# ReplayCoding/mt-renderer

Measured on AMD Instinct MI355X. Metric: Mtris/sec, 1M-tri 64-bone skinned scene @1920x1080, higher is better.
Workload: dtype f32; 1 GPU; headline: 20 x mesh50k primitives = 1,000,000 strip triangles, 506,520 vertices x 24 B, 64-bone palette, debug-id shader, 1920x1080; triangles_per_frame=1000000, collective=none

## Files before the change

### mt_renderer_amd/csrc/k_tile.hip

```cpp
#include "tile_common.h"

namespace mtr {

#define TRI_PASS 64
#ifndef FRAG_K
#define FRAG_K 8u
#endif

struct TriC {
    int32_t A0, B0, C0, A1;
    int32_t B1, C1, A2, B2;
    int32_t C2;
    uint32_t flags;
    float z0, dz1;
    float dz2, rcpA;
    uint32_t rgba8;
    uint32_t pad;
};
struct TriX {
    UVPlanes p;
    uint32_t tw, th, tlevels;
    const uint8_t* tex;
    uint64_t pad2;
};
static_assert(sizeof(TriC) == 64 && sizeof(TriX) == 64, "LDS triangle records are 64 B");
enum { TF_LARGE = 1, TF_TEX = 2, TF_BLEND = 4, TF_ADD = 8, TF_NODW = 128, TF_NODT = 256, TF_BLENDSOLID = 512 };

template <bool TEX>
__device__ __forceinline__ void setup_entry(const TileParams& P, uint32_t r, int32_t binx0, int32_t biny0, TriC& t, TriX* x,
                                            int4& chi, uint32_t& submask) {
    const RecA a = load_rec(P.fb, r);
    const bool solid = (a.pad1 & 1u) != 0;
    DMat mat = {};
    if (!solid) mat = P.mats[a.mat];
    const uint32_t mshader = solid ? (uint32_t)MTR_SH_DEBUG : mat.shader;
    const int32_t X[3] = {a.X0, a.X1, a.X2}, Y[3] = {a.Y0, a.Y1, a.Y2};
    TriSetup g;
    tri_setup(X, Y, a.z0, a.z1, a.z2, binx0, biny0, g);
    uint32_t flags = g.flags;
    if (TEX && mshader == MTR_SH_TEXTURED) flags |= TF_TEX;
    if (!solid) {
        if (mat.blend == MTR_DB_ALPHA) flags |= TF_BLEND;
        if (mat.blend == MTR_DB_ADD) flags |= TF_ADD;
        if (!(mat.dstate & 1u)) flags |= TF_NODW;
        if (!(mat.dstate & 2u)) flags |= TF_NODT;
        if (mshader != MTR_SH_TEXTURED && mat.blend == MTR_DB_ADD) flags |= TF_BLENDSOLID;
    }
    t.A0 = g.A[0]; t.B0 = g.B[0]; t.C0 = g.Clo[0];
    t.A1 = g.A[1]; t.B1 = g.B[1]; t.C1 = g.Clo[1];
    t.A2 = g.A[2]; t.B2 = g.B[2]; t.C2 = g.Clo[2];
    t.flags = flags;
    t.z0 = g.z0; t.dz1 = g.dz1; t.dz2 = g.dz2; t.rcpA = g.rcpA;
    t.rgba8 = solid ? a.pad0 : mat.rgba8;
    chi = make_int4(g.Chi[0], g.Chi[1], g.Chi[2], 0);
// ... 31 lines not shown
    } else {
        const QuadUV q = quad();
        const TexRef tr = {Xt.tex, Xt.tw, Xt.th, Xt.tlevels};
        float src[4];
        sample_texture(tr, q.u, q.v, filter_select(q.dudx, q.dvdx, q.dudy, q.dvdy, tr.tw, tr.th, tr.levels), src);
        col = blend_store(col, src, bmode);
    }
}

template <bool TEX>
__global__ __launch_bounds__(64) void k_tile(TileParams P) {
    __shared__ __align__(16) TriC s_tc[TRI_PASS];
    __shared__ __align__(16) TriX s_tx[TEX ? TRI_PASS : 1];
    __shared__ __align__(16) int4 s_chi[TRI_PASS];
    __shared__ uint32_t s_mask[TRI_PASS];
    __shared__ uint32_t s_off[64], s_pre[65];
    __shared__ Seg s_seg[64];
    __shared__ uint32_t s_cnt[MTR_BIN * MTR_BIN];
    __shared__ __align__(16) uint8_t s_frag[MTR_BIN * MTR_BIN * FRAG_K];
    __shared__ unsigned long long s_start[32];
    __shared__ uint32_t s_pm[TRI_PASS];
    __shared__ uint8_t s_tmap[TRI_PASS];

    const uint32_t ovf = tile_prologue(P);
    const uint32_t lane = threadIdx.x;
    uint32_t bin;
    if (!block_to_bin(P, bin)) return;
    if (P.mixed && !P.bin_flag[bin]) return;
    uint32_t bin_x, bin_y;
    bin_xy(P, bin, bin_x, bin_y);
    const int32_t binx0 = (int32_t)bin_x * MTR_BIN, biny0 = (int32_t)bin_y * MTR_BIN;

    float dep[4];
    uint32_t col[4];
#pragma unroll
    for (int i = 0; i < 4; i++) { dep[i] = P.clear_depth; col[i] = P.clear_rgba8; }
    for (uint32_t i = lane; i < MTR_BIN * MTR_BIN; i += 64) s_cnt[i] = 0u;

    uint32_t seg_lo, S, ent_lo, n_ent;
    bin_queue(P.fb, bin, ent_lo, n_ent, seg_lo, S);
    if (ovf) { n_ent = 0; S = 0; }
    if (P.fb.direct && lane == 0 && n_ent) {
        atomicAdd(&P.fb.counters[MTR_CTR(CTR_ENT, bin)], n_ent);
        atomicAdd(&P.fb.counters[MTR_CTR(CTR_SEG, bin)], S);
    }
    const Seg* segs = P.fb.segs + seg_lo;

    unsigned long long lo = 0, hi = 1ull << 32, width = 1ull << 32, end = 1ull << 32;
    if (S > 64) {
        uint32_t kmin = 0xFFFFFFFFu, kmax = 0;
        for (uint32_t i = lane; i < S; i += 64) { const uint32_t k = segs[i].key; kmin = min(kmin, k); kmax = max(kmax, k); }
#pragma unroll
        for (int d = 32; d > 0; d >>= 1) { kmin = min(kmin, (uint32_t)__shfl_xor((int)kmin, d)); kmax = max(kmax, (uint32_t)__shfl_xor((int)kmax, d)); }
        width = ((unsigned long long)(kmax - kmin) + 1) * 40 / S + 1;
        lo = kmin; hi = lo + width; end = (unsigned long long)kmax + 1;
    }
    while (S != 0 && lo < end) {
        uint32_t n;
        uint32_t mkey = 0xFFFFFFFFu, moff = 0, mcnt = 0;
        if (S <= 64) {
            n = S;
            if (lane < S) { const Seg sg = segs[lane]; mkey = sg.key; moff = sg.off; mcnt = sg.cnt; }
        } else {
            uint32_t cnt = 0;
            for (uint32_t i = lane; i < S; i += 64) { const uint32_t k = segs[i].key; cnt += (k >= lo && k < hi) ? 1u : 0u; }
#pragma unroll
            for (int d = 32; d > 0; d >>= 1) cnt += (uint32_t)__shfl_xor((int)cnt, d);
// ... 31 lines not shown
                }
            uint32_t inc = mcnt;
#pragma unroll
            for (int d = 1; d < 64; d <<= 1) {
                const uint32_t t = (uint32_t)__shfl_up((int)inc, d);
                if ((int)lane >= d) inc += t;
            }
            s_off[lane] = moff;
            s_pre[lane] = inc - mcnt;
            if (lane == 63) s_pre[64] = inc;
            wave_lds_sync();
            const uint32_t N = s_pre[64];

            for (uint32_t e0 = 0; e0 < N; e0 += TRI_PASS) {
                const uint32_t cntp = min((uint32_t)TRI_PASS, N - e0);
                if (lane < cntp) {
                    const uint32_t e = e0 + lane;
                    uint32_t a = 0, b = 64;
#pragma unroll
                    for (int it = 0; it < 6; it++) {
                        const uint32_t mid = (a + b) >> 1;
                        if (s_pre[mid] <= e) a = mid; else b = mid;
                    }
                    const uint32_t ord = P.fb.entries[ent_lo + s_off[a] + (e - s_pre[a])];
                    const uint32_t r = (ord >> 7) * MTR_CHUNK_SLOTS + (ord & 127u);
                    setup_entry<TEX>(P, r, binx0, biny0, s_tc[lane], TEX ? &s_tx[lane] : nullptr, s_chi[lane], s_mask[lane]);
                }
                wave_lds_sync();
                bool listed = false;
                {
                    const uint32_t box = lane < cntp ? s_tc[lane].pad : 0u;
                    const uint32_t bw = ((box >> 8) & 15u) + 1u, bh = ((box >> 12) & 15u) + 1u;
                    const uint32_t mine = (box >> 16) ? bw * bh : 0u;
                    const bool large = lane < cntp && (s_tc[lane].flags & TF_LARGE);
                    const uint32_t inc = wave_incl_scan_u32(mine);
                    const uint32_t total = (uint32_t)__builtin_amdgcn_readlane((int)inc, 63);
                    if (!__ballot(large) && total != 0 && total <= 2048u) {
                        const uint32_t pre = inc - mine, cidx = lane_rank(__ballot(mine != 0));
                        flat_stage_starts(s_start, 32, lane, mine, pre);
                        if (mine) {
                            s_tmap[cidx] = (uint8_t)lane;
                            s_pm[lane] = pre | (row_magic(bw) << 12);
                        }
                        wave_lds_sync();
                        flat_for_each(s_start, 32, lane, total, [&](uint32_t pidx, uint32_t ci) {
                            const uint32_t t = s_tmap[ci];
                            const int4* tc = reinterpret_cast<const int4*>(&s_tc[t]);
// ... 7 lines not shown
                            int32_t e1, e2;
                            if (tri_inside(E, lx, ly, e1, e2)) {
                                const uint32_t pix = (uint32_t)(ly * MTR_BIN + lx);
                                const uint32_t slot = atomicAdd(&s_cnt[pix], 1u);
                                if (slot < FRAG_K) s_frag[pix * FRAG_K + slot] = (uint8_t)t;
                            }
                        });
                        wave_lds_sync();
                        uint32_t cn[4];
                        bool over = false;
#pragma unroll
                        for (int i = 0; i < 4; i++) {
                            const uint32_t pix = (uint32_t)(((i >> 1) * 8 + (lane >> 3)) * MTR_BIN + (i & 1) * 8 + (lane & 7));
                            cn[i] = s_cnt[pix];
                            s_cnt[pix] = 0u;
                            over = over || cn[i] > FRAG_K;
                        }
                        if (!__ballot(over)) {
                            listed = true;
#pragma unroll
                            for (int i = 0; i < 4; i++) {
                                const int32_t lx = (int32_t)((i & 1) * 8 + (lane & 7)), ly = (int32_t)((i >> 1) * 8 + (lane >> 3));
                                const uint32_t pix = (uint32_t)(ly * MTR_BIN + lx);
                                const bool in_vp = (uint32_t)(binx0 + lx) < P.fb.W && (uint32_t)(biny0 + ly) < P.fb.H;
                                uint32_t fw[FRAG_K / 4];
#pragma unroll
                                for (uint32_t j = 0; j < FRAG_K / 4; j++) fw[j] = reinterpret_cast<const uint32_t*>(&s_frag[pix * FRAG_K])[j];
                                const uint32_t n = in_vp ? cn[i] : 0u;
                                int32_t last = -1;
                                for (;;) {
                                    uint32_t best = 255u;
#pragma unroll
                                    for (uint32_t j = 0; j < FRAG_K; j++) {
                                        const uint32_t f = (fw[j >> 2] >> (8u * (j & 3u))) & 0xffu;
                                        if (j < n && (int32_t)f > last && f < best) best = f;
                                    }
                                    if (!__ballot(best != 255u)) break;
                                    if (best == 255u) continue;
                                    last = (int32_t)best;
                                    const int4* tc = reinterpret_cast<const int4*>(&s_tc[best]);
                                    const int4 q0 = tc[0], q1 = tc[1], q2 = tc[2], q3 = tc[3];
                                    const uint32_t flags = (uint32_t)q2.y;
                                    const float rcpA = __int_as_float(q3.y);
                                    auto bary = [&](int32_t x, int32_t y, float& b1, float& b2) {
                                        b1 = tri_bary(tri_edge(q1.y, q0.w, q1.x, x, y), (flags >> 5) & 1u, rcpA);
                                        b2 = tri_bary(tri_edge(q2.x, q1.z, q1.w, x, y), (flags >> 6) & 1u, rcpA);
                                    };
                                    float b1, b2;
                                    bary(lx, ly, b1, b2);
                                    const TriX& Xt = s_tx[TEX ? best : 0];
                                    resolve_fragment<TEX>(q2, q3, Xt, true, b1, b2, dep[i], col[i], [&] { return quad_uv(Xt.p, lx, ly, bary); });
                                }
                            }
                        }
                    }
                }
                if (listed) { wave_lds_sync(); continue; }
#pragma unroll
                for (int i = 0; i < 4; i++) {
                    const int32_t lx = (int32_t)((i & 1) * 8 + (lane & 7)), ly = (int32_t)((i >> 1) * 8 + (lane >> 3));
                    const bool in_vp = (uint32_t)(binx0 + lx) < P.fb.W && (uint32_t)(biny0 + ly) < P.fb.H;
                    uint64_t m = __ballot(lane < cntp && ((s_mask[lane] >> i) & 1u));
                    while (m) {
                        const uint32_t t = __builtin_amdgcn_readfirstlane((uint32_t)__ffsll((long long)m) - 1);
                        m &= m - 1;
                        const int4* tc = reinterpret_cast<const int4*>(&s_tc[t]);
                        const int4 q0 = tc[0], q1 = tc[1], q2 = tc[2], q3 = tc[3];
                        const TriEdges E = {q0.x, q0.y, q0.z, q0.w, q1.x, q1.y, q1.z, q1.w, q2.x};
                        const uint32_t flags = (uint32_t)q2.y;
                        const float rcpA = __int_as_float(q3.y);
                        bool inside;
                        float b1, b2;
                        if (!(flags & TF_LARGE)) {
                            int32_t e1, e2;
                            inside = tri_inside(E, lx, ly, e1, e2);
                            b1 = tri_bary(e1, (flags >> 5) & 1u, rcpA);
                            b2 = tri_bary(e2, (flags >> 6) & 1u, rcpA);
                        } else {
                            const int4 ch = s_chi[t];
                            inside = tri_inside_large(E, ch.x, ch.y, ch.z, flags, rcpA, lx, ly, b1, b2);
                        }
                        const TriX& Xt = s_tx[TEX ? t : 0];
                        QuadUV q = {};
                        if (TEX && (flags & TF_TEX)) {
                            uv_at_bary(Xt.p, b1, b2, q.u, q.v);
                            auto across = [&](float a, uint32_t bit) { return __shfl(a, (int)(lane | bit)) - __shfl(a, (int)(lane & ~bit)); };
                            q.dudx = across(q.u, 1u); q.dvdx = across(q.v, 1u);
                            q.dudy = across(q.u, 8u); q.dvdy = across(q.v, 8u);
                        }
                        resolve_fragment<TEX>(q2, q3, Xt, inside && in_vp, b1, b2, dep[i], col[i], [&] { return q; });
                    }
                }
                wave_lds_sync();
            }
        }
        lo = hi;
        hi = lo + width;
        if (hi > (1ull << 32)) hi = 1ull << 32;
    }

    if (lane == 0) bin_queue_done(P.fb, bin);
#pragma unroll
    for (int i = 0; i < 4; i++) {
        const uint32_t x = (uint32_t)binx0 + (i & 1) * 8 + (lane & 7), y = (uint32_t)biny0 + (i >> 1) * 8 + (lane >> 3);
        if (x < P.fb.W && y < P.fb.H) {
            const size_t pi = (size_t)y * P.fb.W + x;
            reinterpret_cast<uint32_t*>(P.color)[pi] = col[i];
            P.depth[pi] = dep[i];
        }
    }
}

}

void mtr_launch_tile(const TileParams& p_in, bool textured, hipStream_t s) {
    TileParams p = p_in;
    tile_set_divisors(p);
    const uint32_t mine = p.fb.own.own_count;
    if (mine == 0) return;
    uint32_t grid = (mine + 7) / 8 * 8;
    if (p.xcd_run) grid = (grid / 8 + p.xcd_run - 1) / p.xcd_run * p.xcd_run * 8;
    if (textured) hipLaunchKernelGGL(mtr::k_tile<true>, dim3(grid), dim3(64), 0, s, p);
    else hipLaunchKernelGGL(mtr::k_tile<false>, dim3(grid), dim3(64), 0, s, p);
}
```

### mt_renderer_amd/csrc/k_tile_vis.hip

```cpp
#include "tile_common.h"

namespace mtr {

struct VisTri {
    int32_t A0, B0, C0, A1;
    int32_t B1, C1, A2, B2;
    int32_t C2;
    uint32_t flags;
    float z0, dz1;
    float dz2, rcpA;
    uint32_t ordk;
    uint32_t box;
};
static_assert(sizeof(VisTri) == 64, "VisTri is 64 B");

struct Setup {
    VisTri t;
    int4 chi;
    int32_t npx;
    uint32_t bhm1;
};

__device__ __forceinline__ void setup_tri(const RecA& a, uint32_t ord, int32_t binx0, int32_t biny0, int32_t vw, int32_t vh, Setup& s) {
    const int32_t X[3] = {a.X0, a.X1, a.X2}, Y[3] = {a.Y0, a.Y1, a.Y2};
// ... 49 lines not shown
__device__ __forceinline__ float z_at(const RecA& a, int32_t px, int32_t py) {
    float b1, b2;
    tri_abs_bary(a.X0, a.Y0, a.X1, a.Y1, a.X2, a.Y2, px, py, b1, b2);
    return tri_depth(b1, b2, a.z0, a.z1 - a.z0, a.z2 - a.z0);
}

#ifndef VIS_OCC
#define VIS_OCC 6
#endif

template <bool TEX, int VIS_WAVES, bool STAIR, bool QW>
__global__ __launch_bounds__(64 * VIS_WAVES, VIS_OCC) void k_tile_vis(TileParams P) {
    __shared__ unsigned long long s_key[MTR_BIN * MTR_BIN];
    __shared__ uint4 s_flat[VIS_WAVES][64 * 4];
    __shared__ unsigned long long s_start[VIS_WAVES][64];
    __shared__ uint32_t s_trans;
    __shared__ uint32_t s_hard;
    __shared__ uint32_t s_cnt[STAIR ? MTR_BIN * MTR_BIN : 1];
    __shared__ __align__(16) uint32_t s_list[STAIR ? MTR_BIN * MTR_BIN * STAIR_K : 4];

    static_assert(!QW, "the quad walk is retired");
    const uint32_t lane = threadIdx.x & 63;
    const uint32_t wv = __builtin_amdgcn_readfirstlane(threadIdx.x >> 6);
    const uint32_t ovf = tile_prologue(P);
    uint32_t bin;
    if (!block_to_bin(P, bin)) return;
    uint32_t bin_x, bin_y;
    bin_xy(P, bin, bin_x, bin_y);
    const int32_t binx0 = (int32_t)bin_x * MTR_BIN, biny0 = (int32_t)bin_y * MTR_BIN;
    const float cd = P.clear_depth;
    const bool zlim_ok = cd >= 0.0f;
    const uint32_t zlim = __float_as_uint(fminf(cd, 1.0f));
    const int32_t vw = (int32_t)P.fb.W - binx0, vh = (int32_t)P.fb.H - biny0;
    const uint32_t stride = 64 * VIS_WAVES, first = wv * 64;
    uint32_t spec0 = 0, spec1 = 0;
    if (P.fb.direct) {
        const uint32_t qb = bin * P.fb.qcap;
        if (first + lane < P.fb.qcap) spec0 = P.fb.entries[qb + first + lane];
        if (first + stride + lane < P.fb.qcap) spec1 = P.fb.entries[qb + first + stride + lane];
    }
    uint32_t ent_lo, N, seg_lo_unused, n_seg;
    bin_queue(P.fb, bin, ent_lo, N, seg_lo_unused, n_seg);
    if (ovf) {
        N = 0;
        __syncthreads();
        if (threadIdx.x == 0) bin_queue_done(P.fb, bin);
    }
    if (N == 0) {
        for (uint32_t pidx = threadIdx.x; pidx < MTR_BIN * MTR_BIN; pidx += 64 * VIS_WAVES) {
            const int32_t lx = (int32_t)(pidx & (MTR_BIN - 1)), ly = (int32_t)(pidx >> MTR_BIN_SHIFT);
            if (lx >= vw || ly >= vh) continue;
            const size_t pi = (size_t)(biny0 + ly) * P.fb.W + (size_t)(binx0 + lx);
            reinterpret_cast<uint32_t*>(P.color)[pi] = P.clear_rgba8;
            P.depth[pi] = cd;
        }
        if (P.mixed && threadIdx.x == 0) P.bin_flag[bin] = 0;
        if (P.fb.direct && threadIdx.x == 0 && !ovf) P.fb.bin_count[bin] = 0ull;
        return;
    }
    for (uint32_t i = threadIdx.x; i < MTR_BIN * MTR_BIN; i += 64 * VIS_WAVES) {
        s_key[i] = 0ull;
        if (STAIR) s_cnt[i] = 0u;
    }
    if (threadIdx.x == 0) { s_trans = 0u; s_hard = 0u; }
    __syncthreads();

    const RecA zero_rec = {0, 0, 0, 0, 0, 0, 0.0f, 0.0f, 0.0f, 0u, 0u, 0u};
    uint32_t ord_cur = 0, ord_nxt = 0;
    if (P.fb.direct) {
        if (first + lane < N) ord_cur = spec0;
        if (first + stride + lane < N) ord_nxt = spec1;
    } else {
        if (first + lane < N) ord_cur = P.fb.entries[ent_lo + first + lane];
        if (first + stride + lane < N) ord_nxt = P.fb.entries[ent_lo + first + stride + lane];
    }
    RecA a_cur = zero_rec;
    if (first + lane < N) a_cur = load_rec(P.fb, (ord_cur >> 7) * MTR_CHUNK_SLOTS + (ord_cur & 127u));
    for (uint32_t e0 = first; e0 < N; e0 += stride) {
        const bool valid = e0 + lane < N;
        RecA a_nxt = zero_rec;
        if (e0 + stride + lane < N) a_nxt = load_rec(P.fb, (ord_nxt >> 7) * MTR_CHUNK_SLOTS + (ord_nxt & 127u));
        uint32_t ord_nn = 0;
        if (e0 + 2 * stride + lane < N) ord_nn = P.fb.entries[ent_lo + e0 + 2 * stride + lane];

        if (P.mixed && valid && (a_cur.pad1 >> 16)) {
            s_trans = 1u;
            if (!STAIR || (a_cur.pad1 >> 17)) s_hard = 1u;
        }
        Setup s = {};
        if (valid) setup_tri(a_cur, ord_cur, binx0, biny0, vw, vh, s);
        const bool large = (s.t.flags & 1u) != 0;
        const uint32_t iw = ((s.t.box >> 8) & 15u) + 1u;
        const uint32_t npx = (uint32_t)s.npx;
        const uint64_t mlarge = __ballot(npx != 0 && large);
        uint32_t lbox = s.t.box;
        if (mlarge) lbox |= row_magic(iw) << 12;
        for (uint64_t mb = mlarge; mb; mb &= mb - 1) {
            const uint32_t t = __builtin_amdgcn_readfirstlane((uint32_t)__ffsll((long long)mb) - 1);
#define RL(x) __builtin_amdgcn_readlane((int)(x), t)
            const TriEdges E = {RL(s.t.A0), RL(s.t.B0), RL(s.t.C0), RL(s.t.A1), RL(s.t.B1), RL(s.t.C1), RL(s.t.A2), RL(s.t.B2), RL(s.t.C2)};
            const uint32_t flags = (uint32_t)RL(s.t.flags), box = (uint32_t)RL(lbox), tord = (uint32_t)RL(s.t.ordk), tn = (uint32_t)RL(npx);
            const float z0 = __int_as_float(RL(__float_as_int(s.t.z0))), dz1 = __int_as_float(RL(__float_as_int(s.t.dz1)));
            const float dz2 = __int_as_float(RL(__float_as_int(s.t.dz2))), rcpA = __int_as_float(RL(__float_as_int(s.t.rcpA)));
            const int32_t H0 = RL(s.chi.x), H1 = RL(s.chi.y), H2 = RL(s.chi.z);
#undef RL
            const uint32_t bw = ((box >> 8) & 15u) + 1u, magic = box >> 12;
// ... 53 lines not shown
                stage_flat(&s_flat[wv][cidx * 4], s.t, inc - mine);
            }
            wave_lds_sync();
            flat_for_each(s_start[wv], 64, lane, total, [&](uint32_t p, uint32_t tri) {
                const uint4* src = &s_flat[wv][tri * 4];
                const uint4 q0 = src[0], q1 = src[1], q2 = src[2], q3 = src[3];
                const TriEdges E = {(int32_t)q0.x, (int32_t)q0.y, (int32_t)q0.z, (int32_t)q0.w, (int32_t)q1.x, (int32_t)q1.y, (int32_t)q1.z, (int32_t)q1.w, (int32_t)q2.x};
                const uint32_t box = q3.w, k = p - q2.y;
                const int32_t row = (int32_t)((k * ((box >> 12) & 0x1ffffu)) >> 16);
                const int32_t col = (int32_t)k - __mul24(row, (int32_t)((box >> 8) & 15u) + 1);
                int32_t e1, e2;
                const bool inside = tri_inside(E, col, row, e1, e2);
                const float rcpA = __uint_as_float(q3.y);
                const float z = tri_depth(tri_bary(e1, (box >> 29) & 1u, rcpA), tri_bary(e2, (box >> 30) & 1u, rcpA), __uint_as_float(q2.z), __uint_as_float(q2.w),
                                          __uint_as_float(q3.x));
                if (inside && __float_as_uint(z) <= zlim)
                    put_fragment<STAIR>(s_key, s_cnt, s_list, (box & 0xffu) + (uint32_t)(row * MTR_BIN + col), make_key(z, q3.z));
            });
        }
        a_cur = a_nxt;
        ord_cur = ord_nxt;
        ord_nxt = ord_nn;
    }
    __syncthreads();
    bool stair = false;
    if (P.mixed) {
        bool leave = s_hard != 0u;
        if (STAIR && !leave && s_trans) {
            bool over = false;
            for (uint32_t i = threadIdx.x; i < MTR_BIN * MTR_BIN; i += 64 * VIS_WAVES) over = over || s_cnt[i] > STAIR_K;
            leave = __syncthreads_or(over ? 1 : 0) != 0;
            stair = !leave;
        }
        if (threadIdx.x == 0) P.bin_flag[bin] = leave ? 1 : 0;
        if (leave) return;
    }
    if (threadIdx.x == 0) {
        if (P.fb.direct && N) {
            atomicAdd(&P.fb.counters[MTR_CTR(CTR_ENT, bin)], N);
            atomicAdd(&P.fb.counters[MTR_CTR(CTR_SEG, bin)], n_seg);
        }
        bin_queue_done(P.fb, bin);
    }

#pragma unroll
    for (uint32_t pidx = threadIdx.x; pidx < MTR_BIN * MTR_BIN; pidx += 64 * VIS_WAVES) {
        const int32_t lx = (int32_t)(pidx & (MTR_BIN - 1)), ly = (int32_t)(pidx >> MTR_BIN_SHIFT);
        if (lx >= vw || ly >= vh) continue;
        const uint32_t x = (uint32_t)(binx0 + lx), y = (uint32_t)(biny0 + ly);
        const unsigned long long key = s_key[ly * MTR_BIN + lx];
        uint32_t col = P.clear_rgba8;
        float dep = cd;
        if (STAIR && stair) {
            const uint32_t pix = (uint32_t)(ly * MTR_BIN + lx);
            const uint32_t n = s_cnt[pix];
            const uint4 l0 = reinterpret_cast<const uint4*>(&s_list[pix * STAIR_K])[0], l1 = reinterpret_cast<const uint4*>(&s_list[pix * STAIR_K])[1];
            const uint32_t lst[STAIR_K] = {l0.x, l0.y, l0.z, l0.w, l1.x, l1.y, l1.z, l1.w};
            uint32_t last = 0;
            for (;;) {
                uint32_t best = 0xFFFFFFFFu;
#pragma unroll
                for (uint32_t j = 0; j < STAIR_K; j++)
                    if (j < n && lst[j] > last && lst[j] < best) best = lst[j];
                if (best == 0xFFFFFFFFu) break;
                last = best;
                const uint32_t ord = best - 1u;
                const uint32_t r = (ord >> 7) * MTR_CHUNK_SLOTS + (ord & 127u);
                const RecA a = load_rec(P.fb, r);
                const float z = z_at(a, (int32_t)x, (int32_t)y);
                if (!(z <= dep)) continue;
                dep = z;
                if (a.pad1 & 1u) {
                    col = a.pad0;
                } else {
                    const DMat mat = P.mats[a.mat];
                    if (TEX && mat.shader == MTR_SH_TEXTURED) {
                        const RecB b = P.fb.rec_b[r];
                        float src[4];
                        sample_textured(a, b, mat, (int32_t)x, (int32_t)y, src);
                        col = blend_store(col, src, mat.blend == MTR_DB_ALPHA ? 1u : 0u);
                    } else {
                        col = mat.rgba8;
                    }
                }
            }
        } else if (key != 0ull) {
            dep = __uint_as_float(~(uint32_t)(key >> 32));
            const uint32_t ord = (uint32_t)key - 1u;
            const uint32_t r = (ord >> 7) * MTR_CHUNK_SLOTS + (ord & 127u);
            const uint32_t payload = P.fb.rec_a[r].q1.w;
            if ((payload >> 24) != 0xFFu) {
                const DMat mat = P.mats[payload & 0xFFFFFFu];
                if (TEX && mat.shader == MTR_SH_TEXTURED) {
                    const RecA a = load_rec(P.fb, r);
                    const RecB b = P.fb.rec_b[r];
                    float src[4];
                    sample_textured(a, b, mat, (int32_t)x, (int32_t)y, src);
                    col = blend_store(0u, src, 0u);
                } else {
                    col = mat.rgba8;
                }
            } else {
                col = payload;
            }
        }
        const size_t pi = (size_t)y * P.fb.W + x;
        reinterpret_cast<uint32_t*>(P.color)[pi] = col;
        P.depth[pi] = dep;
    }
}

}

void mtr_launch_tile_vis(const TileParams& p_in, bool textured, hipStream_t s) {
    TileParams p = p_in;
    tile_set_divisors(p);
    const uint32_t mine = p.fb.own.own_count;
    if (mine == 0) return;
    uint32_t grid = (mine + 7) / 8 * 8;
    if (p.xcd_run) grid = (grid / 8 + p.xcd_run - 1) / p.xcd_run * p.xcd_run * 8;
    const int waves = (int)mtr_vis_waves_for(p.vis_waves, mine);
#define MTR_LAUNCH_VIS(T, W, S) hipLaunchKernelGGL((mtr::k_tile_vis<T, W, S, false>), dim3(grid), dim3(64 * W), 0, s, p)
#define MTR_LAUNCH_VIS_W(T, S) do { if (waves >= 8) MTR_LAUNCH_VIS(T, 8, S); else if (waves >= 4) MTR_LAUNCH_VIS(T, 4, S); else MTR_LAUNCH_VIS(T, 2, S); } while (0)
    if (p.mixed) { if (textured) MTR_LAUNCH_VIS_W(true, true); else MTR_LAUNCH_VIS_W(false, true); }
    else { if (textured) MTR_LAUNCH_VIS_W(true, false); else MTR_LAUNCH_VIS_W(false, false); }
#undef MTR_LAUNCH_VIS_W
#undef MTR_LAUNCH_VIS
}
```

### mt_renderer_amd/csrc/mtr_internal.h

```cpp
#pragma once
#include <hip/hip_runtime.h>
#include <stdint.h>

#define MTR_BIN 16
#define MTR_BIN_SHIFT 4
#define MTR_SUB 8
#define MTR_CHUNK_NEW 62
#define MTR_CHUNK_SLOTS 124
#define MTR_GUARD_BAND 1048576.0f

enum { MTR_SH_DEBUG = 0, MTR_SH_TEXTURED = 1, MTR_SH_CONST = 2 };

struct DPrim {
    uint32_t vertex_base, vertex_num, stride;
    uint32_t index_ofs, index_num, index_base;
    uint32_t topology;
    uint32_t pos_fmt, pos_cnt, pos_off;
    uint32_t uv_fmt, uv_cnt, uv_off, has_uv;
    uint32_t joint_off, weight_off, skinnable;
    uint32_t aligned4;
    uint32_t parts_no;
    uint32_t cull;
};

// ... 240 lines not shown
    const DChunk* chunks;
    const BoneBox* boxes;
    uint32_t nchunks;
    uint32_t ninst;
    const uint16_t* work_mask;
    uint32_t work_nx;
    uint32_t work_slot_base;
    uint32_t rest_split;
    uint32_t slots_override;
    uint32_t small_draw;
    const uint32_t* inst_list;
    const uint32_t* inst_count;
    uint32_t slots_hint;
    const float* model_mats;
    const float* palettes;
    uint32_t npal, pal_stride;
    float vp[16];
    uint32_t chunk_base;
    uint32_t mat_base, mat_inst_stride;
    const DMat* mats;
    FrameBuffers fb;
};

struct TileParams {
    FrameBuffers fb;
    const DMat* mats;
    uint8_t* color;
    float* depth;
    uint32_t clear_rgba8;
    float clear_depth;
    uint8_t* bin_flag;
    uint32_t mixed;
    uint32_t* zero_next;
    uint32_t* host_status;
    uint32_t vis_waves;
    uint32_t xcd_run;
    uint32_t* zero_words;
    uint32_t zero_nwords;
    uint32_t* hint_out;
    uint32_t nhint;
    uint16_t hint_word[4], hint_slot[4];
    uint32_t nbx_mul, nbx_shift, run_mul, run_shift;
};

static inline uint32_t mtr_vis_waves_for(uint32_t forced, uint32_t own_count) {
    if (forced) return forced;
    return own_count <= 1536 ? 8u : own_count <= 4096 ? 4u : 2u;
}

void mtr_launch_geom(const GeomParams& p, hipStream_t s);
void mtr_launch_scan(const FrameBuffers& fb, hipStream_t s);
void mtr_launch_fill(const FrameBuffers& fb, uint32_t total_chunks, hipStream_t s);
void mtr_launch_tile(const TileParams& p, bool textured, hipStream_t s);
void mtr_launch_tile_vis(const TileParams& p, bool textured, hipStream_t s);
void mtr_launch_alpha_min(const uint8_t* rgba, size_t npixels, uint32_t* out_min, hipStream_t s);
void mtr_launch_vertex_stage(const GeomParams& p, uint32_t prim, float* out_clip, float* out_uv, hipStream_t s);
void mtr_launch_bc1_decode(const uint8_t* blocks, uint8_t* rgba, uint32_t w, uint32_t h, hipStream_t s);
void mtr_launch_bc7_decode(const uint8_t* blocks, uint8_t* rgba, uint32_t w, uint32_t h, hipStream_t s);
void mtr_launch_pack_shard(const uint8_t* color, uint8_t* dst, uint32_t W, uint32_t H, const uint32_t* own_list, uint32_t own_count,
                           uint32_t stride_bins, hipStream_t s);
void mtr_launch_unpack_shards(const uint8_t* gathered, uint8_t* color, uint32_t W, uint32_t H, const uint32_t* src_of_bin, hipStream_t s);
struct CullParams {
    const BoneBox* boxes;
    uint32_t nboxes;
    uint32_t ninst;
    const float* model_mats;
// ... 120 lines not shown
```

### mt_renderer_amd/csrc/tile_common.h

```cpp
#pragma once
#include <cstdint>

#if defined(__HIP_DEVICE_COMPILE__)
#define MTR_UMULHI(a, b) __umulhi((a), (b))
#else
#define MTR_UMULHI(a, b) ((uint32_t)(((uint64_t)(uint32_t)(a) * (uint64_t)(uint32_t)(b)) >> 32))
#endif
#if defined(__HIPCC__)
#include <hip/hip_runtime.h>
#define MTR_DIV_HD __host__ __device__ __forceinline__
#else
#define MTR_DIV_HD inline
#endif

namespace mtr {

struct UDiv {
    uint32_t mul, shift;
};
MTR_DIV_HD UDiv udiv_make(uint32_t d) {
    UDiv r = {0u, 0u};
    if (d == 0u) return r;
    while ((d >> r.shift) > 1u) r.shift++;
    r.mul = (uint32_t)((((uint64_t)1 << (31u + r.shift)) + d - 1u) / d);
    return r;
}
MTR_DIV_HD uint32_t udiv_apply(uint32_t n, uint32_t mul, uint32_t shift) { return MTR_UMULHI(n << 1, mul) >> shift; }

MTR_DIV_HD uint32_t row_magic(uint32_t iw) { return (65536u + iw - 1u) / iw; }

}

#if defined(__HIPCC__)
#include "bc_sample.h"
#include "mtr_internal.h"
#include "span_row.h"

namespace mtr {

__device__ __forceinline__ void zero_next_counters(const TileParams& P) {
    if (P.zero_words)
        for (uint32_t i = blockIdx.x * blockDim.x + threadIdx.x; i < P.zero_nwords; i += gridDim.x * blockDim.x) {
            for (uint32_t k = 0; k < P.nhint; k++)
                if (i - P.hint_word[k] < 2u)
                    __hip_atomic_store(&P.hint_out[2u * P.hint_slot[k] + (i - P.hint_word[k])], 0x80000000u | P.zero_words[i], __ATOMIC_RELAXED,
                                       __HIP_MEMORY_SCOPE_SYSTEM);
            P.zero_words[i] = 0u;
        }
    if (!P.zero_next) return;
    for (uint32_t i = blockIdx.x * blockDim.x + threadIdx.x; i < (uint32_t)CTR_NUM; i += gridDim.x * blockDim.x) P.zero_next[i] = 0u;
}

__device__ __forceinline__ uint32_t tile_prologue(const TileParams& P) {
    zero_next_counters(P);
    const uint32_t ovf = P.fb.counters[CTR_OVERFLOW];
    if (blockIdx.x == 0 && threadIdx.x == 0 && P.host_status)
        __hip_atomic_store(P.host_status, 0x80000000u | ovf, __ATOMIC_RELAXED, __HIP_MEMORY_SCOPE_SYSTEM);
    return ovf;
}

__device__ __forceinline__ RecA load_rec(const FrameBuffers& fb, uint32_t r) {
    const RecP p = fb.rec_a[r];
    int4 l = make_int4(0, 0, 0, 0);
    if ((p.q0.z & 0xFFFFu) == MTR_REC_LARGE_SENTINEL) l = fb.rec_l[r];
    return rec_unpack(p, l);
}

__device__ __forceinline__ float unorm8f(uint32_t v) {
    const float x = (float)(v & 0xffu), r = __uint_as_float(0x3b808081u);
    const float q0 = x * r;
    return fmaf(fmaf(-q0, 255.0f, x), r, q0);
}
__device__ __forceinline__ uint32_t quant8(float x) {
    if (!(x > 0.0f)) x = 0.0f;
    if (x > 1.0f) x = 1.0f;
    return (uint32_t)rintf(x * 255.0f);
}
__device__ __forceinline__ int32_t clamp_texel(float f, uint32_t n) {
    if (!(f >= 0.0f)) f = 0.0f;
    if (f > (float)(n - 1)) f = (float)(n - 1);
    return (int32_t)f;
}
struct TexRef {
    const uint8_t* tex;
    uint32_t tw, th;
    uint32_t levels;
};
// ... 113 lines not shown
}
__device__ __forceinline__ void uv_at_bary(const UVPlanes& p, float b1, float b2, float& u, float& v) {
    const float iw = fmaf(b2, p.diw2, fmaf(b1, p.diw1, p.iw0));
    const float up = fmaf(b2, p.dup2, fmaf(b1, p.dup1, p.up0));
    const float vp = fmaf(b2, p.dvp2, fmaf(b1, p.dvp1, p.vp0));
    u = up / iw;
    v = vp / iw;
}
struct QuadUV { float u, v, dudx, dvdx, dudy, dvdy; };
template <typename B>
__device__ __forceinline__ QuadUV quad_uv(const UVPlanes& p, int32_t x, int32_t y, B&& bary) {
    auto uv_at = [&](int32_t qx, int32_t qy, float& u, float& v) {
        float b1, b2;
        bary(qx, qy, b1, b2);
        uv_at_bary(p, b1, b2, u, v);
    };
    float u, v, uh, vh, uw, vw;
    uv_at(x, y, u, v);
    uv_at(x ^ 1, y, uh, vh);
    uv_at(x, y ^ 1, uw, vw);
    return {u, v, (x & 1) ? u - uh : uh - u, (x & 1) ? v - vh : vh - v, (y & 1) ? u - uw : uw - u, (y & 1) ? v - vw : vw - v};
}

__device__ __forceinline__ bool block_to_bin(const TileParams& P, uint32_t& bin) {
    const FrameBuffers& fb = P.fb;
    const uint32_t run = P.xcd_run;
    const uint32_t per = (gridDim.x + 7) / 8;
    const uint32_t x = blockIdx.x & 7, i = blockIdx.x >> 3;
    uint32_t slot = x * per + i;
    if (run) {
        const uint32_t q = udiv_apply(i, P.run_mul, P.run_shift);
        slot = (q * 8 + x) * run + (i - q * run);
    }
    if (slot >= fb.own.own_count) return false;
    bin = fb.own.own_list ? fb.own.own_list[slot] : slot;
    return bin < fb.nbx * fb.nby;
}
__device__ __forceinline__ void bin_xy(const TileParams& P, uint32_t bin, uint32_t& bx, uint32_t& by) {
    by = udiv_apply(bin, P.nbx_mul, P.nbx_shift);
    bx = bin - by * P.fb.nbx;
}

}

inline void tile_set_divisors(TileParams& p) {
    const mtr::UDiv n = mtr::udiv_make(p.fb.nbx), r = mtr::udiv_make(p.xcd_run);
    p.nbx_mul = n.mul; p.nbx_shift = n.shift;
    p.run_mul = r.mul; p.run_shift = r.shift;
}
#endif
```

Baseline: 22360 Mtris/s.

## Pack hot tile-kernel arguments into a cache-aligned head and reorder prologue loads

Adds a 192-byte, 64-byte-aligned TileHead at the front of the kernel arguments. It holds the scalars and pointers the tile prologue needs, and asm constraints pin them in scalar registers. A new tile_enter issues the bin mapping, overflow counter and queue-bounds loads (plus speculative entry loads) before the counter-zeroing work, so their latency overlaps. Late-use arguments are reloaded from the kernarg segment after the main loop, which aims to cut SGPR pressure across the loop. The cost is extra kernarg size and more complex code, and the gain depends on how prologue latency compares with the tile work.

```diff
diff --git a/mt_renderer_amd/csrc/k_tile.hip b/mt_renderer_amd/csrc/k_tile.hip
--- a/mt_renderer_amd/csrc/k_tile.hip
+++ b/mt_renderer_amd/csrc/k_tile.hip
@@ -29,7 +29,7 @@
 template <bool TEX>
 __device__ __forceinline__ void setup_entry(const TileParams& P, uint32_t r, int32_t binx0, int32_t biny0, TriC& t, TriX* x,
                                             int4& chi, uint32_t& submask) {
-    const RecA a = load_rec(P.fb, r);
+    const RecA a = load_rec(P.fb.rec_a, P.fb.rec_l, r);
     const bool solid = (a.pad1 & 1u) != 0;
     DMat mat = {};
     if (!solid) mat = P.mats[a.mat];
@@ -107,14 +107,13 @@
     __shared__ uint32_t s_pm[TRI_PASS];
     __shared__ uint8_t s_tmap[TRI_PASS];
 
-    const uint32_t ovf = tile_prologue(P);
     const uint32_t lane = threadIdx.x;
-    uint32_t bin;
-    if (!block_to_bin(P, bin)) return;
+    TileEntry te;
+    if (!tile_enter<64, false>(P, 0u, lane, te)) return;
+    const TileHead& hd = te.h;
+    const uint32_t ovf = te.ovf, bin = te.bin;
     if (P.mixed && !P.bin_flag[bin]) return;
-    uint32_t bin_x, bin_y;
-    bin_xy(P, bin, bin_x, bin_y);
-    const int32_t binx0 = (int32_t)bin_x * MTR_BIN, biny0 = (int32_t)bin_y * MTR_BIN;
+    const int32_t binx0 = (int32_t)te.bin_x * MTR_BIN, biny0 = (int32_t)te.bin_y * MTR_BIN;
 
     float dep[4];
     uint32_t col[4];
@@ -122,12 +121,12 @@
     for (int i = 0; i < 4; i++) { dep[i] = P.clear_depth; col[i] = P.clear_rgba8; }
     for (uint32_t i = lane; i < MTR_BIN * MTR_BIN; i += 64) s_cnt[i] = 0u;
 
-    uint32_t seg_lo, S, ent_lo, n_ent;
-    bin_queue(P.fb, bin, ent_lo, n_ent, seg_lo, S);
+    const uint32_t seg_lo = te.seg_lo, ent_lo = te.ent_lo;
+    uint32_t S = te.n_seg, n_ent = te.n_ent;
     if (ovf) { n_ent = 0; S = 0; }
-    if (P.fb.direct && lane == 0 && n_ent) {
-        atomicAdd(&P.fb.counters[MTR_CTR(CTR_ENT, bin)], n_ent);
-        atomicAdd(&P.fb.counters[MTR_CTR(CTR_SEG, bin)], S);
+    if (hd.direct && lane == 0 && n_ent) {
+        atomicAdd(&hd.counters[MTR_CTR(CTR_ENT, bin)], n_ent);
+        atomicAdd(&hd.counters[MTR_CTR(CTR_SEG, bin)], S);
     }
     const Seg* segs = P.fb.segs + seg_lo;
 
@@ -205,7 +204,7 @@
                         const uint32_t mid = (a + b) >> 1;
                         if (s_pre[mid] <= e) a = mid; else b = mid;
                     }
-                    const uint32_t ord = P.fb.entries[ent_lo + s_off[a] + (e - s_pre[a])];
+                    const uint32_t ord = hd.entries[ent_lo + s_off[a] + (e - s_pre[a])];
                     const uint32_t r = (ord >> 7) * MTR_CHUNK_SLOTS + (ord & 127u);
                     setup_entry<TEX>(P, r, binx0, biny0, s_tc[lane], TEX ? &s_tx[lane] : nullptr, s_chi[lane], s_mask[lane]);
                 }
@@ -259,7 +258,7 @@
                             for (int i = 0; i < 4; i++) {
                                 const int32_t lx = (int32_t)((i & 1) * 8 + (lane & 7)), ly = (int32_t)((i >> 1) * 8 + (lane >> 3));
                                 const uint32_t pix = (uint32_t)(ly * MTR_BIN + lx);
-                                const bool in_vp = (uint32_t)(binx0 + lx) < P.fb.W && (uint32_t)(biny0 + ly) < P.fb.H;
+                                const bool in_vp = (uint32_t)(binx0 + lx) < hd.W && (uint32_t)(biny0 + ly) < hd.H;
                                 uint32_t fw[FRAG_K / 4];
 #pragma unroll
                                 for (uint32_t j = 0; j < FRAG_K / 4; j++) fw[j] = reinterpret_cast<const uint32_t*>(&s_frag[pix * FRAG_K])[j];
@@ -296,7 +295,7 @@
 #pragma unroll
                 for (int i = 0; i < 4; i++) {
                     const int32_t lx = (int32_t)((i & 1) * 8 + (lane & 7)), ly = (int32_t)((i >> 1) * 8 + (lane >> 3));
-                    const bool in_vp = (uint32_t)(binx0 + lx) < P.fb.W && (uint32_t)(biny0 + ly) < P.fb.H;
+                    const bool in_vp = (uint32_t)(binx0 + lx) < hd.W && (uint32_t)(biny0 + ly) < hd.H;
                     uint64_t m = __ballot(lane < cntp && ((s_mask[lane] >> i) & 1u));
                     while (m) {
                         const uint32_t t = __builtin_amdgcn_readfirstlane((uint32_t)__ffsll((long long)m) - 1);
@@ -340,8 +339,8 @@
 #pragma unroll
     for (int i = 0; i < 4; i++) {
         const uint32_t x = (uint32_t)binx0 + (i & 1) * 8 + (lane & 7), y = (uint32_t)biny0 + (i >> 1) * 8 + (lane >> 3);
-        if (x < P.fb.W && y < P.fb.H) {
-            const size_t pi = (size_t)y * P.fb.W + x;
+        if (x < hd.W && y < hd.H) {
+            const size_t pi = (size_t)y * hd.W + x;
             reinterpret_cast<uint32_t*>(P.color)[pi] = col[i];
             P.depth[pi] = dep[i];
         }
@@ -352,11 +351,9 @@
 
 void mtr_launch_tile(const TileParams& p_in, bool textured, hipStream_t s) {
     TileParams p = p_in;
-    tile_set_divisors(p);
-    const uint32_t mine = p.fb.own.own_count;
+    tile_fill_head(p);
+    const uint32_t mine = p.fb.own.own_count, grid = p.head.grid;
     if (mine == 0) return;
-    uint32_t grid = (mine + 7) / 8 * 8;
-    if (p.xcd_run) grid = (grid / 8 + p.xcd_run - 1) / p.xcd_run * p.xcd_run * 8;
     if (textured) hipLaunchKernelGGL(mtr::k_tile<true>, dim3(grid), dim3(64), 0, s, p);
     else hipLaunchKernelGGL(mtr::k_tile<false>, dim3(grid), dim3(64), 0, s, p);
 }
diff --git a/mt_renderer_amd/csrc/k_tile_vis.hip b/mt_renderer_amd/csrc/k_tile_vis.hip
--- a/mt_renderer_amd/csrc/k_tile_vis.hip
+++ b/mt_renderer_amd/csrc/k_tile_vis.hip
@@ -95,25 +95,18 @@
     static_assert(!QW, "the quad walk is retired");
     const uint32_t lane = threadIdx.x & 63;
     const uint32_t wv = __builtin_amdgcn_readfirstlane(threadIdx.x >> 6);
-    const uint32_t ovf = tile_prologue(P);
-    uint32_t bin;
-    if (!block_to_bin(P, bin)) return;
-    uint32_t bin_x, bin_y;
-    bin_xy(P, bin, bin_x, bin_y);
-    const int32_t binx0 = (int32_t)bin_x * MTR_BIN, biny0 = (int32_t)bin_y * MTR_BIN;
+    const uint32_t stride = 64 * VIS_WAVES, first = wv * 64;
+    TileEntry te;
+    if (!tile_enter<64 * VIS_WAVES, true>(P, first, lane, te)) return;
+    const TileHead& hd = te.h;
+    const uint32_t ovf = te.ovf, bin = te.bin, ent_lo = te.ent_lo, n_seg = te.n_seg;
+    const uint32_t spec0 = te.spec0, spec1 = te.spec1;
+    uint32_t N = te.n_ent;
+    const int32_t binx0 = (int32_t)te.bin_x * MTR_BIN, biny0 = (int32_t)te.bin_y * MTR_BIN;
     const float cd = P.clear_depth;
     const bool zlim_ok = cd >= 0.0f;
     const uint32_t zlim = __float_as_uint(fminf(cd, 1.0f));
-    const int32_t vw = (int32_t)P.fb.W - binx0, vh = (int32_t)P.fb.H - biny0;
-    const uint32_t stride = 64 * VIS_WAVES, first = wv * 64;
-    uint32_t spec0 = 0, spec1 = 0;
-    if (P.fb.direct) {
-        const uint32_t qb = bin * P.fb.qcap;
-        if (first + lane < P.fb.qcap) spec0 = P.fb.entries[qb + first + lane];
-        if (first + stride + lane < P.fb.qcap) spec1 = P.fb.entries[qb + first + stride + lane];
-    }
-    uint32_t ent_lo, N, seg_lo_unused, n_seg;
-    bin_queue(P.fb, bin, ent_lo, N, seg_lo_unused, n_seg);
+    const int32_t vw = (int32_t)hd.W - binx0, vh = (int32_t)hd.H - biny0;
     if (ovf) {
         N = 0;
         __syncthreads();
@@ -123,38 +116,37 @@
         for (uint32_t pidx = threadIdx.x; pidx < MTR_BIN * MTR_BIN; pidx += 64 * VIS_WAVES) {
             const int32_t lx = (int32_t)(pidx & (MTR_BIN - 1)), ly = (int32_t)(pidx >> MTR_BIN_SHIFT);
             if (lx >= vw || ly >= vh) continue;
-            const size_t pi = (size_t)(biny0 + ly) * P.fb.W + (size_t)(binx0 + lx);
+            const size_t pi = (size_t)(biny0 + ly) * hd.W + (size_t)(binx0 + lx);
             reinterpret_cast<uint32_t*>(P.color)[pi] = P.clear_rgba8;
             P.depth[pi] = cd;
         }
         if (P.mixed && threadIdx.x == 0) P.bin_flag[bin] = 0;
-        if (P.fb.direct && threadIdx.x == 0 && !ovf) P.fb.bin_count[bin] = 0ull;
+        if (hd.direct && threadIdx.x == 0 && !ovf) P.fb.bin_count[bin] = 0ull;
         return;
     }
+    const RecA zero_rec = {0, 0, 0, 0, 0, 0, 0.0f, 0.0f, 0.0f, 0u, 0u, 0u};
+    uint32_t ord_cur = 0, ord_nxt = 0;
+    if (hd.direct) {
+        if (first + lane < N) ord_cur = spec0;
+        if (first + stride + lane < N) ord_nxt = spec1;
+    } else {
+        if (first + lane < N) ord_cur = hd.entries[ent_lo + first + lane];
+        if (first + stride + lane < N) ord_nxt = hd.entries[ent_lo + first + stride + lane];
+    }
+    RecA a_cur = zero_rec;
+    if (first + lane < N) a_cur = load_rec(hd.rec_a, P.fb.rec_l, (ord_cur >> 7) * MTR_CHUNK_SLOTS + (ord_cur & 127u));
     for (uint32_t i = threadIdx.x; i < MTR_BIN * MTR_BIN; i += 64 * VIS_WAVES) {
         s_key[i] = 0ull;
         if (STAIR) s_cnt[i] = 0u;
     }
     if (threadIdx.x == 0) { s_trans = 0u; s_hard = 0u; }
     __syncthreads();
-
-    const RecA zero_rec = {0, 0, 0, 0, 0, 0, 0.0f, 0.0f, 0.0f, 0u, 0u, 0u};
-    uint32_t ord_cur = 0, ord_nxt = 0;
-    if (P.fb.direct) {
-        if (first + lane < N) ord_cur = spec0;
-        if (first + stride + lane < N) ord_nxt = spec1;
-    } else {
-        if (first + lane < N) ord_cur = P.fb.entries[ent_lo + first + lane];
-        if (first + stride + lane < N) ord_nxt = P.fb.entries[ent_lo + first + stride + lane];
-    }
-    RecA a_cur = zero_rec;
-    if (first + lane < N) a_cur = load_rec(P.fb, (ord_cur >> 7) * MTR_CHUNK_SLOTS + (ord_cur & 127u));
     for (uint32_t e0 = first; e0 < N; e0 += stride) {
         const bool valid = e0 + lane < N;
         RecA a_nxt = zero_rec;
-        if (e0 + stride + lane < N) a_nxt = load_rec(P.fb, (ord_nxt >> 7) * MTR_CHUNK_SLOTS + (ord_nxt & 127u));
+        if (e0 + stride + lane < N) a_nxt = load_rec(hd.rec_a, P.fb.rec_l, (ord_nxt >> 7) * MTR_CHUNK_SLOTS + (ord_nxt & 127u));
         uint32_t ord_nn = 0;
-        if (e0 + 2 * stride + lane < N) ord_nn = P.fb.entries[ent_lo + e0 + 2 * stride + lane];
+        if (e0 + 2 * stride + lane < N) ord_nn = hd.entries[ent_lo + e0 + 2 * stride + lane];
 
         if (P.mixed && valid && (a_cur.pad1 >> 16)) {
             s_trans = 1u;
@@ -254,9 +246,10 @@
         ord_cur = ord_nxt;
         ord_nxt = ord_nn;
     }
+    const TileLate Q = tile_late();
     __syncthreads();
     bool stair = false;
-    if (P.mixed) {
+    if (Q.mixed) {
         bool leave = s_hard != 0u;
         if (STAIR && !leave && s_trans) {
             bool over = false;
@@ -264,15 +257,15 @@
             leave = __syncthreads_or(over ? 1 : 0) != 0;
             stair = !leave;
         }
-        if (threadIdx.x == 0) P.bin_flag[bin] = leave ? 1 : 0;
+        if (threadIdx.x == 0) Q.bin_flag[bin] = leave ? 1 : 0;
         if (leave) return;
     }
     if (threadIdx.x == 0) {
-        if (P.fb.direct && N) {
-            atomicAdd(&P.fb.counters[MTR_CTR(CTR_ENT, bin)], N);
-            atomicAdd(&P.fb.counters[MTR_CTR(CTR_SEG, bin)], n_seg);
-        }
-        bin_queue_done(P.fb, bin);
+        if (Q.direct && N) {
+            atomicAdd(&Q.counters[MTR_CTR(CTR_ENT, bin)], N);
+            atomicAdd(&Q.counters[MTR_CTR(CTR_SEG, bin)], n_seg);
+        }
+        bin_queue_done(Q, bin);
     }
 
 #pragma unroll
@@ -281,7 +274,7 @@
         if (lx >= vw || ly >= vh) continue;
         const uint32_t x = (uint32_t)(binx0 + lx), y = (uint32_t)(biny0 + ly);
         const unsigned long long key = s_key[ly * MTR_BIN + lx];
-        uint32_t col = P.clear_rgba8;
+        uint32_t col = Q.clear_rgba8;
         float dep = cd;
         if (STAIR && stair) {
             const uint32_t pix = (uint32_t)(ly * MTR_BIN + lx);
@@ -298,16 +291,16 @@
                 last = best;
                 const uint32_t ord = best - 1u;
                 const uint32_t r = (ord >> 7) * MTR_CHUNK_SLOTS + (ord & 127u);
-                const RecA a = load_rec(P.fb, r);
+                const RecA a = load_rec(Q.rec_a, Q.rec_l, r);
                 const float z = z_at(a, (int32_t)x, (int32_t)y);
                 if (!(z <= dep)) continue;
                 dep = z;
                 if (a.pad1 & 1u) {
                     col = a.pad0;
                 } else {
-                    const DMat mat = P.mats[a.mat];
+                    const DMat mat = Q.mats[a.mat];
                     if (TEX && mat.shader == MTR_SH_TEXTURED) {
-                        const RecB b = P.fb.rec_b[r];
+                        const RecB b = Q.rec_b[r];
                         float src[4];
                         sample_textured(a, b, mat, (int32_t)x, (int32_t)y, src);
                         col = blend_store(col, src, mat.blend == MTR_DB_ALPHA ? 1u : 0u);
@@ -320,12 +313,12 @@
             dep = __uint_as_float(~(uint32_t)(key >> 32));
             const uint32_t ord = (uint32_t)key - 1u;
             const uint32_t r = (ord >> 7) * MTR_CHUNK_SLOTS + (ord & 127u);
-            const uint32_t payload = P.fb.rec_a[r].q1.w;
+            const uint32_t payload = Q.rec_a[r].q1.w;
             if ((payload >> 24) != 0xFFu) {
-                const DMat mat = P.mats[payload & 0xFFFFFFu];
+                const DMat mat = Q.mats[payload & 0xFFFFFFu];
                 if (TEX && mat.shader == MTR_SH_TEXTURED) {
-                    const RecA a = load_rec(P.fb, r);
-                    const RecB b = P.fb.rec_b[r];
+                    const RecA a = load_rec(Q.rec_a, Q.rec_l, r);
+                    const RecB b = Q.rec_b[r];
                     float src[4];
                     sample_textured(a, b, mat, (int32_t)x, (int32_t)y, src);
                     col = blend_store(0u, src, 0u);
@@ -336,9 +329,9 @@
                 col = payload;
             }
         }
-        const size_t pi = (size_t)y * P.fb.W + x;
-        reinterpret_cast<uint32_t*>(P.color)[pi] = col;
-        P.depth[pi] = dep;
+        const size_t pi = (size_t)y * Q.W + x;
+        reinterpret_cast<uint32_t*>(Q.color)[pi] = col;
+        Q.depth[pi] = dep;
     }
 }
 
@@ -346,11 +339,9 @@
 
 void mtr_launch_tile_vis(const TileParams& p_in, bool textured, hipStream_t s) {
     TileParams p = p_in;
-    tile_set_divisors(p);
-    const uint32_t mine = p.fb.own.own_count;
+    tile_fill_head(p);
+    const uint32_t mine = p.fb.own.own_count, grid = p.head.grid;
     if (mine == 0) return;
-    uint32_t grid = (mine + 7) / 8 * 8;
-    if (p.xcd_run) grid = (grid / 8 + p.xcd_run - 1) / p.xcd_run * p.xcd_run * 8;
     const int waves = (int)mtr_vis_waves_for(p.vis_waves, mine);
 #define MTR_LAUNCH_VIS(T, W, S) hipLaunchKernelGGL((mtr::k_tile_vis<T, W, S, false>), dim3(grid), dim3(64 * W), 0, s, p)
 #define MTR_LAUNCH_VIS_W(T, S) do { if (waves >= 8) MTR_LAUNCH_VIS(T, 8, S); else if (waves >= 4) MTR_LAUNCH_VIS(T, 4, S); else MTR_LAUNCH_VIS(T, 2, S); } while (0)
diff --git a/mt_renderer_amd/csrc/mtr_internal.h b/mt_renderer_amd/csrc/mtr_internal.h
--- a/mt_renderer_amd/csrc/mtr_internal.h
+++ b/mt_renderer_amd/csrc/mtr_internal.h
@@ -286,7 +286,30 @@
     FrameBuffers fb;
 };
 
+struct alignas(64) TileHead {
+    uint32_t grid;
+    uint32_t own_count;
+    uint32_t nbx, nbins;
+    uint32_t W, H;
+    uint32_t direct, qcap, scap;
+    uint32_t xcd_run;
+    uint32_t nbx_mul, nbx_shift, run_mul, run_shift;
+    uint32_t zero_nwords, nhint;
+    const uint32_t* own_list;
+    uint32_t* entries;
+    unsigned long long* bin_fill;
+    uint32_t* bin_start;
+    uint32_t* seg_start;
+    uint32_t* counters;
+    RecP* rec_a;
+    uint32_t* zero_next;
+    uint32_t* zero_words;
+    uint32_t* host_status;
+};
+static_assert(sizeof(TileHead) == 192 && alignof(TileHead) == 64, "TileHead is three 64-byte lines");
+
 struct TileParams {
+    TileHead head;
     FrameBuffers fb;
     const DMat* mats;
     uint8_t* color;
@@ -304,8 +327,8 @@
     uint32_t* hint_out;
     uint32_t nhint;
     uint16_t hint_word[4], hint_slot[4];
-    uint32_t nbx_mul, nbx_shift, run_mul, run_shift;
-};
+};
+#define MTR_TILE_PARAMS 1
 
 static inline uint32_t mtr_vis_waves_for(uint32_t forced, uint32_t own_count) {
     if (forced) return forced;
diff --git a/mt_renderer_amd/csrc/tile_common.h b/mt_renderer_amd/csrc/tile_common.h
--- a/mt_renderer_amd/csrc/tile_common.h
+++ b/mt_renderer_amd/csrc/tile_common.h
@@ -38,31 +38,68 @@
 
 namespace mtr {
 
-__device__ __forceinline__ void zero_next_counters(const TileParams& P) {
-    if (P.zero_words)
-        for (uint32_t i = blockIdx.x * blockDim.x + threadIdx.x; i < P.zero_nwords; i += gridDim.x * blockDim.x) {
-            for (uint32_t k = 0; k < P.nhint; k++)
-                if (i - P.hint_word[k] < 2u)
-                    __hip_atomic_store(&P.hint_out[2u * P.hint_slot[k] + (i - P.hint_word[k])], 0x80000000u | P.zero_words[i], __ATOMIC_RELAXED,
-                                       __HIP_MEMORY_SCOPE_SYSTEM);
-            P.zero_words[i] = 0u;
+__device__ __forceinline__ TileHead tile_head(const TileParams& P) {
+    const TileHead h = P.head;
+    asm volatile("" ::"s"(h.grid), "s"(h.own_count), "s"(h.nbx), "s"(h.nbins), "s"(h.W), "s"(h.H), "s"(h.direct), "s"(h.qcap), "s"(h.scap),
+                 "s"(h.xcd_run), "s"(h.nbx_mul), "s"(h.nbx_shift), "s"(h.run_mul), "s"(h.run_shift), "s"(h.zero_nwords), "s"(h.nhint),
+                 "s"(h.own_list), "s"(h.entries), "s"(h.bin_fill), "s"(h.bin_start), "s"(h.seg_start), "s"(h.counters), "s"(h.rec_a),
+                 "s"(h.zero_next), "s"(h.zero_words), "s"(h.host_status));
+    return h;
+}
+
+template <uint32_t BLOCK>
+__device__ __forceinline__ void zero_next_counters(const TileParams& P, const TileHead& h) {
+    const uint32_t b0 = blockIdx.x * BLOCK, step = h.grid * BLOCK;
+    if (h.zero_words && b0 < h.zero_nwords) {
+        const auto pack4 = [](const uint16_t (&a)[4]) { return (uint64_t)a[0] | (uint64_t)a[1] << 16 | (uint64_t)a[2] << 32 | (uint64_t)a[3] << 48; };
+        const uint64_t hint_words = pack4(P.hint_word), hint_slots = pack4(P.hint_slot);
+        for (uint32_t i = b0 + threadIdx.x; i < h.zero_nwords; i += step) {
+            for (uint32_t k = 0; k < h.nhint; k++) {
+                const uint32_t hw = (uint32_t)(hint_words >> (16u * k)) & 0xffffu, hs = (uint32_t)(hint_slots >> (16u * k)) & 0xffffu;
+                if (i - hw < 2u)
+                    __hip_atomic_store(&P.hint_out[2u * hs + (i - hw)], 0x80000000u | h.zero_words[i], __ATOMIC_RELAXED, __HIP_MEMORY_SCOPE_SYSTEM);
+            }
+            h.zero_words[i] = 0u;
         }
-    if (!P.zero_next) return;
-    for (uint32_t i = blockIdx.x * blockDim.x + threadIdx.x; i < (uint32_t)CTR_NUM; i += gridDim.x * blockDim.x) P.zero_next[i] = 0u;
-}
-
-__device__ __forceinline__ uint32_t tile_prologue(const TileParams& P) {
-    zero_next_counters(P);
-    const uint32_t ovf = P.fb.counters[CTR_OVERFLOW];
-    if (blockIdx.x == 0 && threadIdx.x == 0 && P.host_status)
-        __hip_atomic_store(P.host_status, 0x80000000u | ovf, __ATOMIC_RELAXED, __HIP_MEMORY_SCOPE_SYSTEM);
-    return ovf;
-}
-
-__device__ __forceinline__ RecA load_rec(const FrameBuffers& fb, uint32_t r) {
-    const RecP p = fb.rec_a[r];
+    }
+    if (h.zero_next && b0 < (uint32_t)CTR_NUM)
+        for (uint32_t i = b0 + threadIdx.x; i < (uint32_t)CTR_NUM; i += step) h.zero_next[i] = 0u;
+}
+
+struct TileLate {
+    const DMat* mats;
+    uint8_t* color;
+    float* depth;
+    uint8_t* bin_flag;
+    RecP* rec_a;
+    int4* rec_l;
+    RecB* rec_b;
+    unsigned long long* bin_count;
+    unsigned long long* bin_fill;
+    uint32_t* counters;
+    uint32_t W, clear_rgba8, mixed, direct;
+};
+__device__ __forceinline__ TileLate tile_late() {
+    typedef const TileParams __attribute__((address_space(4)))* TileArgs;
+    TileArgs q = (TileArgs)__builtin_amdgcn_kernarg_segment_ptr();
+    asm volatile("" : "+s"(q));
+    const TileLate t = {q->mats,         q->color,        q->depth,       q->bin_flag, q->fb.rec_a,    q->fb.rec_l, q->fb.rec_b,
+                        q->fb.bin_count, q->fb.bin_fill,  q->fb.counters, q->fb.W,     q->clear_rgba8, q->mixed,    q->fb.direct};
+    asm volatile("" ::"s"(t.mats), "s"(t.color), "s"(t.depth), "s"(t.bin_flag), "s"(t.rec_a), "s"(t.rec_l), "s"(t.rec_b), "s"(t.bin_count),
+                 "s"(t.bin_fill), "s"(t.counters), "s"(t.W), "s"(t.clear_rgba8), "s"(t.mixed), "s"(t.direct));
+    return t;
+}
+__device__ __forceinline__ void bin_queue_done(const TileLate& t, uint32_t bin) {
+    if (t.direct) {
+        t.bin_count[bin] = t.bin_fill[bin];
+        t.bin_fill[bin] = 0ull;
+    }
+}
+
+__device__ __forceinline__ RecA load_rec(const RecP* rec_a, const int4* rec_l, uint32_t r) {
+    const RecP p = rec_a[r];
     int4 l = make_int4(0, 0, 0, 0);
-    if ((p.q0.z & 0xFFFFu) == MTR_REC_LARGE_SENTINEL) l = fb.rec_l[r];
+    if ((p.q0.z & 0xFFFFu) == MTR_REC_LARGE_SENTINEL) l = rec_l[r];
     return rec_unpack(p, l);
 }
 
@@ -222,30 +259,92 @@
     return {u, v, (x & 1) ? u - uh : uh - u, (x & 1) ? v - vh : vh - v, (y & 1) ? u - uw : uw - u, (y & 1) ? v - vw : vw - v};
 }
 
-__device__ __forceinline__ bool block_to_bin(const TileParams& P, uint32_t& bin) {
-    const FrameBuffers& fb = P.fb;
-    const uint32_t run = P.xcd_run;
-    const uint32_t per = (gridDim.x + 7) / 8;
+__device__ __forceinline__ bool block_to_bin(const TileHead& h, uint32_t& bin) {
+    const uint32_t run = h.xcd_run;
+    const uint32_t per = (h.grid + 7) / 8;
     const uint32_t x = blockIdx.x & 7, i = blockIdx.x >> 3;
     uint32_t slot = x * per + i;
     if (run) {
-        const uint32_t q = udiv_apply(i, P.run_mul, P.run_shift);
+        const uint32_t q = udiv_apply(i, h.run_mul, h.run_shift);
         slot = (q * 8 + x) * run + (i - q * run);
     }
-    if (slot >= fb.own.own_count) return false;
-    bin = fb.own.own_list ? fb.own.own_list[slot] : slot;
-    return bin < fb.nbx * fb.nby;
-}
-__device__ __forceinline__ void bin_xy(const TileParams& P, uint32_t bin, uint32_t& bx, uint32_t& by) {
-    by = udiv_apply(bin, P.nbx_mul, P.nbx_shift);
-    bx = bin - by * P.fb.nbx;
-}
-
-}
-
-inline void tile_set_divisors(TileParams& p) {
+    bin = 0;
+    if (slot >= h.own_count) return false;
+    bin = h.own_list ? h.own_list[slot] : slot;
+    return bin < h.nbins;
+}
+__device__ __forceinline__ void bin_xy(const TileHead& h, uint32_t bin, uint32_t& bx, uint32_t& by) {
+    by = udiv_apply(bin, h.nbx_mul, h.nbx_shift);
+    bx = bin - by * h.nbx;
+}
+
+struct TileEntry {
+    TileHead h;
+    uint32_t ovf, bin, bin_x, bin_y;
+    uint32_t ent_lo, n_ent, seg_lo, n_seg;
+    uint32_t spec0, spec1;
+};
+template <uint32_t BLOCK, bool SPEC>
+__device__ __forceinline__ bool tile_enter(const TileParams& P, uint32_t first, uint32_t lane, TileEntry& e) {
+    e.h = tile_head(P);
+    const TileHead& h = e.h;
+    const bool has_bin = block_to_bin(h, e.bin);
+    const uint32_t bin = e.bin;
+    const uint32_t ovf_v = h.counters[CTR_OVERFLOW];
+    unsigned long long fill = 0ull;
+    uint32_t e0 = 0, e1 = 0, s0 = 0, s1 = 0;
+    e.spec0 = e.spec1 = 0u;
+    if (has_bin) {
+        if (h.direct) {
+            fill = h.bin_fill[bin];
+            if (SPEC) {
+                const uint32_t qb = bin * h.qcap;
+                if (first + lane < h.qcap) e.spec0 = h.entries[qb + first + lane];
+                if (first + BLOCK + lane < h.qcap) e.spec1 = h.entries[qb + first + BLOCK + lane];
+            }
+        } else {
+            e0 = h.bin_start[bin]; e1 = h.bin_start[bin + 1];
+            s0 = h.seg_start[bin]; s1 = h.seg_start[bin + 1];
+        }
+    }
+    zero_next_counters<BLOCK>(P, h);
+    if (blockIdx.x == 0 && threadIdx.x == 0 && h.host_status)
+        __hip_atomic_store(h.host_status, 0x80000000u | ovf_v, __ATOMIC_RELAXED, __HIP_MEMORY_SCOPE_SYSTEM);
+    if (!has_bin) return false;
+    bin_xy(h, bin, e.bin_x, e.bin_y);
+    const auto uni = [](uint32_t v) { return (uint32_t)__builtin_amdgcn_readfirstlane((int)v); };
+    e.ovf = uni(ovf_v);
+    if (h.direct) {
+        e.ent_lo = bin * h.qcap; e.seg_lo = bin * h.scap;
+        e.n_ent = min(uni((uint32_t)fill), h.qcap); e.n_seg = min(uni((uint32_t)(fill >> 32)), h.scap);
+    } else {
+        e.ent_lo = uni(e0); e.n_ent = uni(e1) - e.ent_lo;
+        e.seg_lo = uni(s0); e.n_seg = uni(s1) - e.seg_lo;
+    }
+    return true;
+}
+
+}
+
+#endif
+
+#if defined(MTR_TILE_PARAMS)
+inline void tile_fill_head(TileParams& p) {
+    TileHead& h = p.head;
+    const uint32_t mine = p.fb.own.own_count;
+    h.grid = (mine + 7) / 8 * 8;
+    if (p.xcd_run) h.grid = (h.grid / 8 + p.xcd_run - 1) / p.xcd_run * p.xcd_run * 8;
+    h.own_count = mine; h.own_list = p.fb.own.own_list;
+    h.nbx = p.fb.nbx; h.nbins = p.fb.nbx * p.fb.nby;
+    h.W = p.fb.W; h.H = p.fb.H;
+    h.direct = p.fb.direct; h.qcap = p.fb.qcap; h.scap = p.fb.scap;
+    h.xcd_run = p.xcd_run;
     const mtr::UDiv n = mtr::udiv_make(p.fb.nbx), r = mtr::udiv_make(p.xcd_run);
-    p.nbx_mul = n.mul; p.nbx_shift = n.shift;
-    p.run_mul = r.mul; p.run_shift = r.shift;
+    h.nbx_mul = n.mul; h.nbx_shift = n.shift;
+    h.run_mul = r.mul; h.run_shift = r.shift;
+    h.zero_nwords = p.zero_nwords; h.nhint = p.nhint;
+    h.entries = p.fb.entries; h.bin_fill = p.fb.bin_fill; h.bin_start = p.fb.bin_start; h.seg_start = p.fb.seg_start;
+    h.counters = p.fb.counters; h.rec_a = p.fb.rec_a;
+    h.zero_next = p.zero_next; h.zero_words = p.zero_words; h.host_status = p.host_status;
 }
 #endif
```

Result: faster. 23390 Mtris/s (median of 6 runs) (+4.6%).
